# syzhang092218-source/dgppo

Hardware: AMD Instinct MI355X
Metric: env-steps/sec whole node, LidarSpread n=8 4096 envs, 1/2/4/8 GPUs (higher is better)
Workload: dtype f32

## Files before the change

### dgppo_amd/csrc/nn_dense.hip

```cpp
#include "common.h"

using f32x4 = __attribute__((ext_vector_type(4))) float;
#ifdef DGPPO_STAMPS
__device__ unsigned long long g_dstamps[32];
#define DSTAMP(i) do { if (blockIdx.x == 0 && threadIdx.x == 0) g_dstamps[i] = __builtin_amdgcn_s_memtime(); } while (0)
extern "C" int32_t dgppo_debug_stamps_dense(unsigned long long* out) {
  return (int32_t)hipMemcpyFromSymbol(out, HIP_SYMBOL(g_dstamps), sizeof(unsigned long long) * 32);
}
#else
#define DSTAMP(i)
#endif

#define DENSE_ROWS 64

struct DenseArgs {
  const float* X; int ldx;
  const float* W; int ldw;
  const float* bias;
  float* Y; int ldy;
  int M, K, N;
  int act;
  int accumulate;
  int trans_w;
  const float* mask; int ldm;
// ... 335 lines not shown
}

struct DenseBwdWArgs {
  const float* X; int ldx;
  const float* dY; int ldy;
  float* dW; int ldw;
  float* db;
  int M, K, N;
  int rows_per_block;
  float* part;
  int part_stride;
  size_t ws_bytes;
};

#define BW_ROWS 32
template <int NT, int KT>
__global__ void __launch_bounds__(256) dense_bwd_w_kernel(DenseBwdWArgs a) {
  extern __shared__ float sm[];
  constexpr int KTW = (KT + 3) / 4;
  constexpr int Kl = (KT & 1) ? KT * 16 : KT * 16 + 16;
  constexpr int Nl = (NT & 1) ? NT * 16 : NT * 16 + 16;
  constexpr int BUF = BW_ROWS * (Kl + Nl);
  constexpr int XQ = KT * 4, YQ = NT * 4;
  constexpr int PFX = (BW_ROWS * XQ + 255) / 256, PFY = (BW_ROWS * YQ + 255) / 256;
  const int K = a.K, N = a.N;
  const int tid = threadIdx.x, lane = tid & 63, wave = tid >> 6;
  const int li = lane & 15, lq = lane >> 4;
  const int m_begin = blockIdx.x * a.rows_per_block;
  const int m_end = min(a.M, m_begin + a.rows_per_block);
  const bool vec = ((K & 3) == 0) && ((a.ldx & 3) == 0) && ((reinterpret_cast<uintptr_t>(a.X) & 15) == 0) &&
                   ((N & 3) == 0) && ((a.ldy & 3) == 0) && ((reinterpret_cast<uintptr_t>(a.dY) & 15) == 0);
  const int K4 = K >> 2, N4 = N >> 2;
  f32x4 acc[KTW][NT];
#pragma unroll
  for (int i = 0; i < KTW; ++i)
#pragma unroll
    for (int t = 0; t < NT; ++t) acc[i][t] = f32x4{0.f, 0.f, 0.f, 0.f};
  float4 pfx[PFX], pfy[PFY], csum[PFY];
#pragma unroll
  for (int u = 0; u < PFY; ++u) csum[u] = make_float4(0.f, 0.f, 0.f, 0.f);

  auto fetch = [&](int m0) {
#pragma unroll
    for (int u = 0; u < PFX; ++u) {
// ... 62 lines not shown
        av[i] = xs[s4 * 4 * Kl + kt * 16];
      }
#pragma unroll
      for (int i = 0; i < KTW; ++i)
#pragma unroll
        for (int t = 0; t < NT; ++t) acc[i][t] = __builtin_amdgcn_mfma_f32_16x16x4f32(av[i], bv[t], acc[i][t], 0, 0, 0);
    }
  };
#define DGPPO_LDS_BARRIER() asm volatile("s_waitcnt lgkmcnt(0)\n\ts_barrier" ::: "memory")
  float colsum = 0.0f;
  if (vec) {
    fetch(m_begin);
    commit(m_begin, 0);
    __syncthreads();
    int cur = 0;
    for (int m0 = m_begin; m0 < m_end; m0 += BW_ROWS) {
      fetch(m0 + BW_ROWS);
      __builtin_amdgcn_sched_barrier(0);
      compute(cur);
      commit(m0 + BW_ROWS, cur ^ 1);
      DGPPO_LDS_BARRIER();
      cur ^= 1;
    }
  } else {
    for (int m0 = m_begin; m0 < m_end; m0 += BW_ROWS) {
      stage_scalar(m0);
      __syncthreads();
      if (a.db != nullptr && tid < N) {
        const float* ys = sm + BW_ROWS * Kl;
        float cs = 0.0f;
#pragma unroll 8
        for (int r = 0; r < BW_ROWS; ++r) cs += ys[r * Nl + tid];
        colsum += cs;
      }
      compute(0);
      __syncthreads();
    }
  }
#undef DGPPO_LDS_BARRIER
  float* slab = a.part ? a.part + (size_t)blockIdx.x * a.part_stride : nullptr;
#pragma unroll
  for (int i = 0; i < KTW; ++i) {
    const int kt = wave + 4 * i;
    if (kt >= KT) continue;
#pragma unroll
    for (int t = 0; t < NT; ++t) {
      const int col = t * 16 + li;
      if (col >= N) continue;
#pragma unroll
      for (int r = 0; r < 4; ++r) {
        const int krow = kt * 16 + lq * 4 + r;
        if (krow >= K) continue;
        if (slab) slab[krow * N + col] = acc[i][t][r];
        else atomicAdd(a.dW + (size_t)krow * a.ldw + col, acc[i][t][r]);
      }
    }
  }
  if (a.db != nullptr) {
    float cs = colsum;
// ... 1 lines not shown
      __syncthreads();
      float* red = sm;
#pragma unroll
      for (int u = 0; u < PFY; ++u) {
        const int idx = u * 256 + tid;
        const int r = idx / YQ, q = idx - r * YQ;
        if (idx < BW_ROWS * YQ) *reinterpret_cast<float4*>(red + r * (YQ * 4) + 4 * q) = csum[u];
      }
      __syncthreads();
      cs = 0.0f;
      if (tid < N) {
#pragma unroll 8
        for (int r = 0; r < BW_ROWS; ++r) cs += red[r * (YQ * 4) + tid];
      }
    }
    if (tid < N) {
      if (slab) slab[K * N + tid] = cs;
      else atomicAdd(a.db + tid, cs);
    }
  }
}

__global__ void __launch_bounds__(256) dense_bwd_w_reduce_kernel(const float* __restrict__ part, int part_stride, int G,
                                                                 float* __restrict__ dW, int ldw, float* __restrict__ db,
                                                                 int K, int N) {
  const int e = blockIdx.x * 256 + threadIdx.x;
  const int E = K * N + (db ? N : 0);
  if (e >= E) return;
  const int per = (G + gridDim.y - 1) / gridDim.y;
  const int g0 = blockIdx.y * per, g1 = min(G, g0 + per);
  float s0 = 0.f, s1 = 0.f, s2 = 0.f, s3 = 0.f;
  int g = g0;
  for (; g + 3 < g1; g += 4) {
    s0 += part[(size_t)g * part_stride + e];
    s1 += part[(size_t)(g + 1) * part_stride + e];
    s2 += part[(size_t)(g + 2) * part_stride + e];
// ... 11 lines not shown
}

static thread_local dgppo_reduce_desc* g_defer = nullptr;

struct ReduceBatch {
  int n;
  dgppo_reduce_desc d[DGPPO_REDUCE_BATCH];
};

__global__ void __launch_bounds__(256) dense_bwd_w_reduce_batch_kernel(ReduceBatch b) {
  const dgppo_reduce_desc& d = b.d[blockIdx.z];
  const int K = d.K, N = d.N, G = d.slabs;
  const int e = blockIdx.x * 256 + threadIdx.x;
  const int E = K * N + (d.db ? N : 0);
  if (e >= E) return;
  const int splits = min((int)gridDim.y, max(1, (G + 31) / 32));
  if ((int)blockIdx.y >= splits) return;
  const int per = (G + splits - 1) / splits;
  const int g0 = blockIdx.y * per, g1 = min(G, g0 + per);
  if (g0 >= g1) return;
  const float* part = d.part;
  const size_t st = (size_t)d.part_stride;
  float s0 = 0.f, s1 = 0.f, s2 = 0.f, s3 = 0.f;
  int g = g0;
  for (; g + 3 < g1; g += 4) {
    s0 += part[(size_t)g * st + e]; s1 += part[(size_t)(g + 1) * st + e];
    s2 += part[(size_t)(g + 2) * st + e]; s3 += part[(size_t)(g + 3) * st + e];
  }
  for (; g < g1; ++g) s0 += part[(size_t)g * st + e];
  const float sum = (s0 + s1) + (s2 + s3);
  if (e < K * N) {
    const int k = e / N, n = e - k * N;
    atomicAdd(d.dW + (size_t)k * d.ldw + n, sum);
  } else {
    atomicAdd(d.db + (e - K * N), sum);
  }
}

static void reduce_or_defer(hipStream_t s, const float* part, int stride, int grid, float* dW, int ldw, float* db, int K, int N) {
  if (g_defer != nullptr) {
    dgppo_reduce_desc& d = *g_defer;
    d.part = part; d.part_stride = stride; d.slabs = grid; d.dW = dW; d.ldw = ldw; d.db = db; d.K = K; d.N = N; d.pending = 1;
    return;
  }
  const int E = K * N + (db ? N : 0);
  int splits = cdiv(grid, 32);
  splits = splits < 1 ? 1 : (splits > 64 ? 64 : splits);
  hipLaunchKernelGGL(dense_bwd_w_reduce_kernel, dim3(cdiv(E, 256), splits), dim3(256), 0, s, part, stride, grid, dW, ldw, db, K, N);
}

template <int NT, int KT>
static void launch_bwd_w_kt(DenseBwdWArgs a, hipStream_t s) {
  constexpr int Kl = (KT & 1) ? KT * 16 : KT * 16 + 16;
  constexpr int Nl = (NT & 1) ? NT * 16 : NT * 16 + 16;
  constexpr size_t smem = 2 * sizeof(float) * BW_ROWS * (Kl + Nl);
  static_assert(smem <= 160 * 1024, "dense_bwd_w tiles exceed the 160 KB LDS of a gfx950 CU");
  static thread_local int cap = 0;
  if (cap == 0) {
    int per_cu = 0, dev = 0, cus = 256;
    if (smem > 64 * 1024)
      (void)hipFuncSetAttribute(reinterpret_cast<const void*>(&dense_bwd_w_kernel<NT, KT>),
                                hipFuncAttributeMaxDynamicSharedMemorySize, (int)smem);
    if (hipOccupancyMaxActiveBlocksPerMultiprocessor(&per_cu, reinterpret_cast<const void*>(
            &dense_bwd_w_kernel<NT, KT>), 256, smem) != hipSuccess || per_cu < 1) per_cu = 1;
    if (hipGetDevice(&dev) != hipSuccess ||
        hipDeviceGetAttribute(&cus, hipDeviceAttributeMultiprocessorCount, dev) != hipSuccess || cus < 1) cus = 256;
    cap = per_cu * cus;
  }
  int rpb = cdiv(a.M, cap);
  rpb = ((rpb + BW_ROWS - 1) / BW_ROWS) * BW_ROWS;
  if (rpb < 2 * BW_ROWS) rpb = 2 * BW_ROWS;
  const int stride = ((a.K * a.N + a.N + 63) / 64) * 64;
  const size_t ws_bytes = a.ws_bytes;
  float* ws = cdiv(a.M, rpb) > 4 ? a.part : nullptr;
  if (ws) {
    const long max_slabs = (long)(ws_bytes / (sizeof(float) * stride));
    if (max_slabs < 8) ws = nullptr;
    else if (cdiv(a.M, rpb) > max_slabs) rpb = ((cdiv(a.M, (int)max_slabs) + BW_ROWS - 1) / BW_ROWS) * BW_ROWS;
  }
  a.rows_per_block = rpb;
  a.part = ws;
  a.part_stride = stride;
  const int grid = cdiv(a.M, rpb);
  hipLaunchKernelGGL((dense_bwd_w_kernel<NT, KT>), dim3(grid), dim3(256), smem, s, a);
  if (ws) reduce_or_defer(s, ws, stride, grid, a.dW, a.ldw, a.db, a.K, a.N);
}

template <int NT>
static void launch_bwd_w(const DenseBwdWArgs& a, hipStream_t s) {
  const int kt = cdiv(a.K, 16);
  if (kt <= 1) launch_bwd_w_kt<NT, 1>(a, s);
  else if (kt == 2) launch_bwd_w_kt<NT, 2>(a, s);
  else if (kt == 3) launch_bwd_w_kt<NT, 3>(a, s);
  else if (kt == 4) launch_bwd_w_kt<NT, 4>(a, s);
  else if (kt <= 6) launch_bwd_w_kt<NT, 6>(a, s);
  else if (kt <= 8) launch_bwd_w_kt<NT, 8>(a, s);
  else if (kt == 9) launch_bwd_w_kt<NT, 9>(a, s);
  else if (kt <= 12) launch_bwd_w_kt<NT, 12>(a, s);
  else launch_bwd_w_kt<NT, 16>(a, s);
// ... 109 lines not shown
  DGPPO_REQUIRE(a.N <= 192 && a.K <= 256, "dense_bwd_w: N <= 192 and K <= 256 supported (N=%d K=%d)", a.N, a.K);
  DGPPO_REQUIRE(a.X && a.dY && a.dW, "dense_bwd_w: NULL operand");
  DGPPO_REQUIRE(a.ldx >= a.K && a.ldy >= a.N && a.ldw >= a.N, "dense_bwd_w: leading dimensions too small");
  if (a.M == 0) return 0;
  const int nt = cdiv(a.N, 16);
  if (launch_bwd_w_smallk(a, s)) {}
  else if (nt <= 1) launch_bwd_w<1>(a, s);
  else if (nt <= 2) launch_bwd_w<2>(a, s);
  else if (nt <= 4) launch_bwd_w<4>(a, s);
  else if (nt <= 6) launch_bwd_w<6>(a, s);
  else launch_bwd_w<12>(a, s);
  DGPPO_LAUNCH_CHECK();
  return 0;
}

extern "C" int32_t dgppo_dense_fwd(const float* X, int32_t ldx, const float* W, int32_t ldw, const float* bias, float* Y,
                                   int32_t ldy, int32_t M, int32_t K, int32_t N, int32_t act, int32_t accumulate,
                                   int32_t trans_w, const float* relu_mask, int32_t ldm, void* stream) {
  DGPPO_REQUIRE(relu_mask == nullptr || ldm >= N, "dense: mask leading dimension too small");
  DenseArgs a{X, ldx, W, ldw, bias, Y, ldy, M, K, N, act, accumulate, trans_w, relu_mask, ldm};
  return dense_fwd_launch(a, (hipStream_t)stream);
}

extern "C" int32_t dgppo_dense_bwd_w(const float* X, int32_t ldx, const float* dY, int32_t ldy, float* dW, int32_t ldw,
                                     float* db, int32_t M, int32_t K, int32_t N, float* workspace, int64_t workspace_bytes,
                                     void* stream) {
  DGPPO_REQUIRE(workspace_bytes >= 0 && (workspace != nullptr || workspace_bytes == 0), "dense_bwd_w: bad workspace");
  DGPPO_REQUIRE((reinterpret_cast<uintptr_t>(workspace) & 15) == 0, "dense_bwd_w: workspace must be 16-byte aligned");
  DenseBwdWArgs a{X, ldx, dY, ldy, dW, ldw, db, M, K, N, 0, workspace, 0, (size_t)workspace_bytes};
  return dense_bwd_w_launch(a, (hipStream_t)stream);
// ... 17 lines not shown
  DGPPO_REQUIRE(n >= 0 && (n == 0 || descs != nullptr), "dense_bwd_w_reduce_batch: bad arguments");
  for (int32_t i0 = 0; i0 < n; i0 += DGPPO_REDUCE_BATCH) {
    ReduceBatch b;
    b.n = 0;
    int emax = 0, gmax = 0;
    for (int32_t i = i0; i < n && b.n < DGPPO_REDUCE_BATCH; ++i) {
      if (!descs[i].pending) continue;
      DGPPO_REQUIRE(descs[i].part && descs[i].dW && descs[i].slabs >= 1 && descs[i].K >= 1 && descs[i].N >= 1,
                    "dense_bwd_w_reduce_batch: bad descriptor %d", i);
      b.d[b.n++] = descs[i];
      const int E = descs[i].K * descs[i].N + (descs[i].db ? descs[i].N : 0);
      emax = E > emax ? E : emax;
      gmax = descs[i].slabs > gmax ? descs[i].slabs : gmax;
    }
    if (b.n == 0) continue;
    int splits = cdiv(gmax, 32);
    splits = splits < 1 ? 1 : (splits > 64 ? 64 : splits);
    hipLaunchKernelGGL(dense_bwd_w_reduce_batch_kernel, dim3(cdiv(emax, 256), splits, b.n), dim3(256), 0, (hipStream_t)stream, b);
  }
  DGPPO_LAUNCH_CHECK();
  return 0;
}

extern "C" int64_t dgppo_dense_bwd_w_workspace_bytes(int32_t K, int32_t N) {
  if (K < 1 || N < 1) return 0;
  const int64_t stride = (((int64_t)K * N + N + 63) / 64) * 64;
  return stride * 1024 * (int64_t)sizeof(float);
}
```

### dgppo_amd/csrc/nn_elem.hip

```cpp
#include "common.h"

using f32x4 = __attribute__((ext_vector_type(4))) float;

__device__ inline float wave_sum(float v) {
#pragma unroll
  for (int o = 32; o >= 1; o >>= 1) v += __shfl_xor(v, o);
  return v;
}
template <int NV>
__device__ inline void block_atomic_sums(const float (&v)[NV], float* dst) {
  __shared__ float s_red[4][NV];
  const int lane = threadIdx.x & 63, wave = threadIdx.x >> 6;
#pragma unroll
  for (int k = 0; k < NV; ++k) {
    const float w = wave_sum(v[k]);
    if (lane == 0) s_red[wave][k] = w;
  }
  __syncthreads();
  if (threadIdx.x < NV) {
    float t = 0.0f;
    for (int w = 0; w < (int)(blockDim.x >> 6); ++w) t += s_red[w][threadIdx.x];
    atomicAdd(dst + threadIdx.x, t);
  }
}
// ... 108 lines not shown
#define GRU_H 64
#define GRU_WL 194
#define GRU_HL 66

struct GruArgs {
  const float* gi;
  const float* Wh;
  const float* bhn;
  const float* h0;
  float* hs;
  float* hprev;
  float* gates;
  const float* dhs;
  float* dgi;
  float* dgh;
  int n_seq, T, n_inner;
};

__device__ inline size_t gru_row(const GruArgs& a, int s, int tau) {
  const int grp = s / a.n_inner, i = s - grp * a.n_inner;
  return ((size_t)grp * a.T + tau) * a.n_inner + i;
}
__device__ inline float sigmoidf_(float x) { return 1.0f / (1.0f + expf(-x)); }
__device__ inline float gate_sigmoid(float x) { return __builtin_amdgcn_rcpf(1.0f + __expf(-x)); }
__device__ inline float gate_tanh(float x) { return fmaf(2.0f, __builtin_amdgcn_rcpf(1.0f + __expf(-2.0f * x)), -1.0f); }


#define GRU_LDS_BARRIER() asm volatile("s_waitcnt lgkmcnt(0)\n\ts_barrier" ::: "memory")

template <int RTW>
// ... 112 lines not shown
              float* gs = a.gates + row * 256;
              gs[c] = rg; gs[64 + c] = zg; gs[128 + c] = ng; gs[192 + c] = hn;
            }
          }
        }
      GRU_LDS_BARRIER();
      cur ^= 1;
    }
    if (nxt < n_tiles) {
      commit_h0(sm + cur * (RB * GRU_HL));
      GRU_LDS_BARRIER();
    }
  }
}

template <int RTW>
__global__ void __launch_bounds__(256) gru_bwd_kernel(GruArgs a) {
  extern __shared__ float sm[];
  constexpr int RB = 16 * RTW;
  const int tid = threadIdx.x, lane = tid & 63, w = tid >> 6, li = lane & 15, lq = lane >> 4;
  const int c = w * 16 + li;
  float breg[48];
#pragma unroll
  for (int kk = 0; kk < 48; ++kk) breg[kk] = a.Wh[(size_t)c * 192 + kk * 4 + lq];
  const int n_tiles = (a.n_seq + RB - 1) / RB;
  int cur = 0;
  for (int tile = blockIdx.x; tile < n_tiles; tile += gridDim.x) {
    const int s0 = tile * RB;
    int row0[RTW][4];
    bool ok[RTW][4];
#pragma unroll
// ... 36 lines not shown
          const float d = ok[rt][r] ? dh[rt][r] + du[rt][r] : 0.0f;
          const float dz = d * (hp[rt][r] - ng[rt][r]);
          const float dn = d * (1.0f - zg[rt][r]);
          const float dan = dn * (1.0f - ng[rt][r] * ng[rt][r]);
          const float dhn = dan * rg[rt][r];
          const float dar = dan * hn[rt][r] * rg[rt][r] * (1.0f - rg[rt][r]);
          const float daz = dz * zg[rt][r] * (1.0f - zg[rt][r]);
          dh[rt][r] = d * zg[rt][r];
          s_g[rl * GRU_WL + c] = dar;
          s_g[rl * GRU_WL + 64 + c] = daz;
          s_g[rl * GRU_WL + 128 + c] = dhn;
          if (ok[rt][r]) {
            const size_t row = (size_t)(row0[rt][r] + tau * a.n_inner);
            float* o = a.dgi + row * 192 + c;
            o[0] = dar; o[64] = daz; o[128] = dan;
            float* p = a.dgh + row * 192 + c;
            p[0] = dar; p[64] = daz; p[128] = dhn;
          }
        }
      GRU_LDS_BARRIER();
      if (tau > 0) fetch(tau - 1);
      __builtin_amdgcn_sched_barrier(0);
      f32x4 acc[RTW];
#pragma unroll
      for (int rt = 0; rt < RTW; ++rt) acc[rt] = f32x4{0.f, 0.f, 0.f, 0.f};
#pragma unroll
      for (int k0 = 0; k0 < 48; k0 += 16) {
        float areg[RTW][16];
#pragma unroll
        for (int rt = 0; rt < RTW; ++rt)
#pragma unroll
          for (int u = 0; u < 16; ++u) areg[rt][u] = s_g[(rt * 16 + li) * GRU_WL + (k0 + u) * 4 + lq];
// ... 41 lines not shown
    static thread_local int cap = 0;
    if (cap == 0) cap = gru_resident(reinterpret_cast<const void*>(&gru_fwd_kernel<2>), smem);
    const int tiles = cdiv(n_seq, 32);
    hipLaunchKernelGGL(gru_fwd_kernel<2>, dim3(tiles < cap ? tiles : cap), dim3(256), smem, (hipStream_t)stream, a);
  } else {
    const size_t smem = sizeof(float) * 2 * 16 * GRU_HL;
    static thread_local int cap = 0;
    if (cap == 0) cap = gru_resident(reinterpret_cast<const void*>(&gru_fwd_kernel<1>), smem);
    const int tiles = cdiv(n_seq, 16);
    hipLaunchKernelGGL(gru_fwd_kernel<1>, dim3(tiles < cap ? tiles : cap), dim3(256), smem, (hipStream_t)stream, a);
  }
  DGPPO_LAUNCH_CHECK();
  return 0;
}

extern "C" int32_t dgppo_gru_bwd(const float* dhs, const float* Wh, const float* hprev, const float* gates, float* dgi,
                                 float* dgh, int32_t n_seq, int32_t T, int32_t n_inner, void* stream) {
  GruArgs a{};
  a.dhs = dhs; a.Wh = Wh; a.hprev = (float*)hprev; a.gates = (float*)gates; a.dgi = dgi; a.dgh = dgh;
  a.n_seq = n_seq; a.T = T; a.n_inner = n_inner;
  int32_t rc = gru_check(a);
  if (rc) return rc;
  if (n_seq == 0) return 0;
  DGPPO_REQUIRE(dhs && Wh && hprev && gates && dgi && dgh, "gru_bwd: NULL operand");
  if (cdiv(n_seq, 32) >= 512) {
    const size_t smem = sizeof(float) * 2 * 32 * GRU_WL;
    static thread_local int cap = 0;
    if (cap == 0) cap = gru_resident(reinterpret_cast<const void*>(&gru_bwd_kernel<2>), smem);
    const int tiles = cdiv(n_seq, 32);
    hipLaunchKernelGGL(gru_bwd_kernel<2>, dim3(tiles < cap ? tiles : cap), dim3(256), smem, (hipStream_t)stream, a);
  } else {
    const size_t smem = sizeof(float) * 2 * 16 * GRU_WL;
    static thread_local int cap = 0;
    if (cap == 0) cap = gru_resident(reinterpret_cast<const void*>(&gru_bwd_kernel<1>), smem);
    const int tiles = cdiv(n_seq, 16);
    hipLaunchKernelGGL(gru_bwd_kernel<1>, dim3(tiles < cap ? tiles : cap), dim3(256), smem, (hipStream_t)stream, a);
  }
  DGPPO_LAUNCH_CHECK();
  return 0;
}

#define STD_INIT_INV (-0.43275212956718856f)
#define STD_MIN 1e-5f
#define THRESH 0.999f
#define INV_THRESH 3.8002011672502f
#define LOG_EPS (-6.907755278982137f)
#define HALF_LOG_2PI 0.9189385332046727f
#define LOG2_F 0.6931471805599453f

__device__ inline float softplusf_(float x) { return (x > 20.0f) ? x : log1pf(expf(x)); }
#define NDTR_SERIES_BELOW (-10.0f)
__device__ inline float ndtr_tail_series(float z2) { return 1.0f - 1.0f / z2 + 3.0f / (z2 * z2) - 15.0f / (z2 * z2 * z2); }
__device__ inline float log_ndtrf_(float z) {
  if (z > NDTR_SERIES_BELOW) return logf(0.5f * erfcf(-z * 0.70710678118654752f));
// ... 215 lines not shown
```

### dgppo_amd/nets.py

```python
from __future__ import annotations

import math
from typing import Dict, List, Optional, Tuple

import numpy as np
import torch

from . import _native as N
from . import ops_nn as K

H_HEADS = 3
MSG_DIM = 32
OUT_DIM = 64
HID = 64


def _ceil4(x):
    return (x + 3) // 4 * 4


class Layout:
    def __init__(self):
        self.entries: Dict[str, Tuple[int, Tuple[int, ...]]] = {}
        self.size = 0
# ... 240 lines not shown
                saves = tuple(A.get(f"{tag}.{nm}{i}", Rh, w) for i in (1, 2) for nm, w in (("p", HID), ("y", HID), ("st", 2)))
                for i in (1, 2):
                    act[f"p{i}"], act[f"y{i}"], act[f"st{i}"] = saves[3 * (i - 1):3 * i]
            K.mlp_gi_fwd(x, self.p("mlp.W1"), self.p("mlp.b1"), self.p("mlp.g1"), self.p("mlp.be1"), self.p("mlp.W2"),
                         self.p("mlp.b2"), self.p("mlp.g2"), self.p("mlp.be2"), self.p("gru.Wi"), self.p("gru.bi"), gi, saves)
        assert n_seq * T == Rh, (n_seq, T, Rh)
        L, CD = self.rnn_layers, self.carry_dim
        if h0 is not None:
            assert tuple(h0.shape) == (n_seq, CD), (tuple(h0.shape), n_seq, CD)
        if hs_out is not None:
            assert tuple(hs_out.shape) == (Rh, CD), (tuple(hs_out.shape), Rh, CD)
        act["gi"] = gi
        simple = (self.rnn == "gru" and L == 1)
        if simple:
            hs = hs_out if hs_out is not None else A.get(f"{tag}.hs", Rh, HID)
            hprev = A.get(f"{tag}.hprev", Rh, HID) if train else None
            gates = A.get(f"{tag}.gates", Rh, 4 * HID) if train else None
            feat = hs
            act["hs"], act["hprev"], act["gates"] = hs, hprev, gates
        fused_tail = (simple and T == 1 and self.kind == "policy")
        if simple and not fused_tail:
            K.gru_fwd(gi, self.p("gru.Wh"), self.p("gru.bhn"), h0, hs, hprev, gates, n_seq, T, n_inner)
        if self.rnn == "none":
            feat = act["y2"]
            if hs_out is not None:
                if h0 is not None and T == 1:
                    hs_out.copy_(h0)
                else:
                    hs_out.zero_()
        elif self.rnn == "lstm":
            x_l = act["y2"]
            act["stack"] = []
            for l in range(L):
                zi = A.get(f"{tag}.zi{l}", Rh, 4 * HID)
                for half in (slice(0, 2 * HID), slice(2 * HID, 4 * HID)):
                    K.dense_fwd(x_l, self.p(f"lstm{l}.Wi")[:, half], None, zi[:, half])
                c0_l = h0_l = None
# ... 101 lines not shown
        elif self.rnn == "lstm":
            stack = act["stack"]
            for l in range(len(stack) - 1, -1, -1):
                st = stack[l]
                dz = A.get(f"{tag}.dz_lstm{l}", Rh, 4 * HID)
                K.lstm_bwd(dhs, self.p(f"lstm{l}.Wh"), st["cprev"], st["gates"], dz, n_seq, T, n_inner)
                for half in (slice(0, 2 * HID), slice(2 * HID, 4 * HID)):
                    K.dense_bwd_w(st["hprev"], dz[:, half], self.g(f"lstm{l}.Wh")[:, half], self.g(f"lstm{l}.bh")[half])
                    K.dense_bwd_w(st["x"], dz[:, half], self.g(f"lstm{l}.Wi")[:, half], None)
                dx = A.get(f"{tag}.dy" if l == 0 else f"{tag}.dx{l}", Rh, HID)
                K.dense_fwd(dz, self.p(f"lstm{l}.Wi"), None, dx, trans_w=True)
                dhs = dx
            dy = dhs
        else:
            stack = act.get("stack") or [dict(x=None, gi=act["gi"], hs=act["hs"], hprev=act["hprev"], gates=act["gates"])]
            for l in range(len(stack) - 1, -1, -1):
                st = stack[l]
                pre = "gru" if l == 0 else f"gru{l}"
                dgi = A.get(f"{tag}.dgi{l}", Rh, 3 * HID)
                dgh = A.get(f"{tag}.dgh{l}", Rh, 3 * HID)
                K.gru_bwd(dhs, self.p(f"{pre}.Wh"), st["hprev"], st["gates"], dgi, dgh, n_seq, T, n_inner)
                K.dense_bwd_w(st["hprev"], dgh[:, :2 * HID], self.g(f"{pre}.Wh")[:, :2 * HID], None)
                K.dense_bwd_w(st["hprev"], dgh[:, 2 * HID:], self.g(f"{pre}.Wh")[:, 2 * HID:], self.g(f"{pre}.bhn"))
                x_l = act["y2"] if l == 0 else st["x"]
                K.dense_bwd_w(x_l, dgi, self.g(f"{pre}.Wi"), self.g(f"{pre}.bi"))
                if l == 0 and fused_trunk:
                    dgi0 = dgi
                    break
                dx = A.get(f"{tag}.dy" if l == 0 else f"{tag}.dx{l}", Rh, HID)
                K.dense_fwd(dgi, self.p(f"{pre}.Wi"), None, dx, trans_w=True)
# ... 152 lines not shown
```

### dgppo_amd/ops_nn.py

```python
from __future__ import annotations

import ctypes as C
from typing import Optional

import torch

from . import _native as N

FLOPS = [0.0]


def _mat(t: torch.Tensor, name: str):
    if t.dim() != 2:
        raise ValueError(f"{name} must be 2-D, got {tuple(t.shape)}")
    if not t.is_cuda:
        raise RuntimeError(f"{name} must live on the GPU (the HIP path has no CPU fallback)")
    if t.dtype != torch.float32:
        raise TypeError(f"{name} must be float32")
    if t.shape[1] > 1 and t.stride(1) != 1:
        raise ValueError(f"{name} must have unit inner stride")
    ld = t.stride(0) if t.shape[0] > 1 else max(t.shape[1], t.stride(0))
    return C.c_void_p(t.data_ptr()), int(ld), int(t.shape[0]), int(t.shape[1])


# ... 353 lines not shown
    rc = N.lib().dgppo_gru_fwd(_p(gi), _p(Wh), _p(bhn), _p(h0), _p(hs), _p(hprev), _p(gates), n_seq, T, n_inner,
                               N.stream_ptr())
    N.check(rc, "dgppo_gru_fwd")


def gru_bwd(dhs, Wh, hprev, gates, dgi, dgh, n_seq, T, n_inner):
    rows = n_seq * T
    N.expect_shape(dhs, (rows, 64), "dhs")
    N.expect_shape(dgi, (rows, 192), "dgi")
    N.expect_shape(dgh, (rows, 192), "dgh")
    FLOPS[0] += 2.0 * rows * 64 * 192
    rc = N.lib().dgppo_gru_bwd(_p(dhs), _p(Wh), _p(hprev), _p(gates), _p(dgi), _p(dgh), n_seq, T, n_inner, N.stream_ptr())
    N.check(rc, "dgppo_gru_bwd")


def policy_head(ms, eps, action_in, action, log_pi, entropy, n_agents, mode, log_pi_old=None, adv=None, dms=None,
                stats=None, clip_eps=0.25, coef_ent=0.01):
    rows = ms.shape[0]
    N.expect_shape(ms, (rows, 4), "ms")
    rc = N.lib().dgppo_policy_head(_p(ms), _p(eps), _p(action_in), _p(action), _p(log_pi), _p(entropy), rows, n_agents,
                                   mode, _p(log_pi_old), _p(adv), _p(dms), _p(stats), C.c_float(clip_eps),
                                   C.c_float(coef_ent), N.stream_ptr())
    N.check(rc, "dgppo_policy_head")


def value_loss(v, target, dv, stats):
    rc = N.lib().dgppo_value_loss(_p(v), _p(target), _p(dv), _p(stats), v.numel(), N.stream_ptr())
    N.check(rc, "dgppo_value_loss")


# ... 30 lines not shown
```

### include/dgppo_hip.h

```cpp
#ifndef DGPPO_HIP_H
#define DGPPO_HIP_H

#include <stdint.h>

#ifdef __cplusplus
extern "C" {
#endif

#define DGPPO_ABI_VERSION 3

enum {
  DGPPO_ENV_LIDAR_SPREAD = 0,
  DGPPO_ENV_LIDAR_TARGET = 1,
  DGPPO_ENV_LIDAR_BICYCLE_TARGET = 2,
  DGPPO_ENV_MPE_SPREAD = 3,
  DGPPO_ENV_MPE_TARGET = 4,
  DGPPO_ENV_LIDAR_LINE = 5,
  DGPPO_ENV_MPE_LINE = 6,
  DGPPO_ENV_MPE_FORMATION = 7,
  DGPPO_ENV_MPE_CORRIDOR = 8,
  DGPPO_ENV_MPE_CONNECT_SPREAD = 9,
  DGPPO_ENV_VMAS_REVERSE_TRANSPORT = 10
};
enum {
// ... 149 lines not shown
                       const float* We, const float* Wu, float* Mcat, float* cvec, float* Wout, int32_t F, int32_t Fp,
                       int32_t D, int32_t H, int32_t Kp, void* stream);
int32_t dgppo_gnn_unprep(const float* dMcat, const float* dcvec, const float* dWout, const float* Wq, const float* bq,
                         const float* Wk, float* dWq, float* dbq, float* dWk, float* dWv, float* dbv, float* dWe,
                         float* dWu, int32_t F, int32_t Fp, int32_t D, int32_t H, int32_t Kp, void* stream);

int32_t dgppo_ln_relu_fwd(const float* x, const float* gamma, const float* beta, float* y, float* stats, int32_t M,
                          void* stream);
int32_t dgppo_ln_relu_bwd(const float* x, const float* y, const float* stats, const float* gamma, const float* dy,
                          float* dx, float* dgamma, float* dbeta, int32_t M, void* stream);

int32_t dgppo_gru_fwd(const float* gi, const float* Wh, const float* bhn, const float* h0, float* hs, float* hprev,
                      float* gates, int32_t n_seq, int32_t T, int32_t n_inner, void* stream);
int32_t dgppo_gru_bwd(const float* dhs, const float* Wh, const float* hprev, const float* gates, float* dgi,
                      float* dgh, int32_t n_seq, int32_t T, int32_t n_inner, void* stream);

int32_t dgppo_lstm_fwd(const float* zi, const float* Wh, const float* bh, const float* c0, const float* h0, float* cs,
                       float* hs, float* cprev, float* hprev, float* gates, int32_t n_seq, int32_t T, int32_t n_inner,
                       void* stream);
int32_t dgppo_lstm_bwd(const float* dhs, const float* Wh, const float* cprev, const float* gates, float* dz,
                       int32_t n_seq, int32_t T, int32_t n_inner, void* stream);

int32_t dgppo_policy_head(const float* ms, const float* eps, const float* action_in, float* action, float* log_pi,
                          float* entropy, int32_t rows, int32_t n_agents, int32_t mode, const float* log_pi_old,
                          const float* adv, float* dms, float* stats, float clip_eps, float coef_ent, void* stream);

int32_t dgppo_value_loss(const float* v, const float* target, float* dv, float* stats, int32_t count, void* stream);
int32_t dgppo_mean_agents(const float* x, float* y, int32_t G, int32_t n, int32_t D, int32_t backward,
                          const float* relu_mask, void* stream);
int32_t dgppo_relu_bwd(float* dy, const float* y, int64_t count, void* stream);
// ... 36 lines not shown
```

Measured before the change: 4.004 million.

## Add fused GRU weight-gradient kernel, multi-group bwd_w blocks, and reuse h0 as hprev

Adds a dedicated GRU backward weight-gradient kernel that computes dWi, dWh and both bias gradients in one pass from x, hprev, dgi and dhn. It also adds a dhn-only GRU backward variant feeding it, so the separate dense weight-gradient launches for the GRU go away. The generic dense_bwd_w kernel can now pack several 256-thread groups per workgroup and combine their partials through LDS before writing slabs, which cuts the number of partial slabs to reduce. The reduce split size is halved, and when T==1 the stored hprev buffer is replaced by aliasing h0. This adds code paths and LDS pressure, and moves floating-point summation order.

```diff
diff --git a/dgppo_amd/csrc/nn_dense.hip b/dgppo_amd/csrc/nn_dense.hip
--- a/dgppo_amd/csrc/nn_dense.hip
+++ b/dgppo_amd/csrc/nn_dense.hip
@@ -373,9 +373,9 @@
 };
 
 #define BW_ROWS 32
-template <int NT, int KT>
-__global__ void __launch_bounds__(256) dense_bwd_w_kernel(DenseBwdWArgs a) {
-  extern __shared__ float sm[];
+template <int NT, int KT, int NG>
+__global__ void __launch_bounds__(256 * NG) dense_bwd_w_kernel(DenseBwdWArgs a) {
+  extern __shared__ float sm_wg[];
   constexpr int KTW = (KT + 3) / 4;
   constexpr int Kl = (KT & 1) ? KT * 16 : KT * 16 + 16;
   constexpr int Nl = (NT & 1) ? NT * 16 : NT * 16 + 16;
@@ -383,10 +383,14 @@
   constexpr int XQ = KT * 4, YQ = NT * 4;
   constexpr int PFX = (BW_ROWS * XQ + 255) / 256, PFY = (BW_ROWS * YQ + 255) / 256;
   const int K = a.K, N = a.N;
-  const int tid = threadIdx.x, lane = tid & 63, wave = tid >> 6;
+  const int grp = NG > 1 ? (int)(threadIdx.x >> 8) : 0;
+  const int tid = threadIdx.x & 255, lane = tid & 63, wave = tid >> 6;
   const int li = lane & 15, lq = lane >> 4;
-  const int m_begin = blockIdx.x * a.rows_per_block;
+  float* sm = sm_wg + grp * 2 * BUF;
+  const int wg_begin = blockIdx.x * NG * a.rows_per_block;
+  const int m_begin = wg_begin + grp * a.rows_per_block;
   const int m_end = min(a.M, m_begin + a.rows_per_block);
+  const int n_tiles = (min(a.M - wg_begin, a.rows_per_block) + BW_ROWS - 1) / BW_ROWS;
   const bool vec = ((K & 3) == 0) && ((a.ldx & 3) == 0) && ((reinterpret_cast<uintptr_t>(a.X) & 15) == 0) &&
                    ((N & 3) == 0) && ((a.ldy & 3) == 0) && ((reinterpret_cast<uintptr_t>(a.dY) & 15) == 0);
   const int K4 = K >> 2, N4 = N >> 2;
@@ -479,7 +483,7 @@
     commit(m_begin, 0);
     __syncthreads();
     int cur = 0;
-    for (int m0 = m_begin; m0 < m_end; m0 += BW_ROWS) {
+    for (int it = 0, m0 = m_begin; it < n_tiles; ++it, m0 += BW_ROWS) {
       fetch(m0 + BW_ROWS);
       __builtin_amdgcn_sched_barrier(0);
       compute(cur);
@@ -488,7 +492,7 @@
       cur ^= 1;
     }
   } else {
-    for (int m0 = m_begin; m0 < m_end; m0 += BW_ROWS) {
+    for (int it = 0, m0 = m_begin; it < n_tiles; ++it, m0 += BW_ROWS) {
       stage_scalar(m0);
       __syncthreads();
       if (a.db != nullptr && tid < N) {
@@ -503,11 +507,50 @@
     }
   }
 #undef DGPPO_LDS_BARRIER
+  if (NG > 1) {
+    constexpr int ACCF = KTW * NT * 4 * 256;
+    static_assert(NG == 1 || ACCF + PFY * 4 * 256 <= 2 * BUF, "dense_bwd_w: the group exchange does not fit the tile buffers");
+    __syncthreads();
+    if (grp > 0) {
+#pragma unroll
+      for (int i = 0; i < KTW; ++i)
+#pragma unroll
+        for (int t = 0; t < NT; ++t)
+#pragma unroll
+          for (int r = 0; r < 4; ++r) sm[((i * NT + t) * 4 + r) * 256 + tid] = acc[i][t][r];
+      if (!vec) csum[0].x = colsum;
+#pragma unroll
+      for (int u = 0; u < PFY; ++u) {
+        sm[ACCF + (u * 4 + 0) * 256 + tid] = csum[u].x; sm[ACCF + (u * 4 + 1) * 256 + tid] = csum[u].y;
+        sm[ACCF + (u * 4 + 2) * 256 + tid] = csum[u].z; sm[ACCF + (u * 4 + 3) * 256 + tid] = csum[u].w;
+      }
+    }
+    __syncthreads();
+    if (grp == 0) {
+      for (int g = 1; g < NG; ++g) {
+        const float* o = sm_wg + g * 2 * BUF;
+#pragma unroll
+        for (int i = 0; i < KTW; ++i)
+#pragma unroll
+          for (int t = 0; t < NT; ++t)
+#pragma unroll
+            for (int r = 0; r < 4; ++r) acc[i][t][r] += o[((i * NT + t) * 4 + r) * 256 + tid];
+        if (!vec) colsum += o[ACCF + tid];
+        else {
+#pragma unroll
+          for (int u = 0; u < PFY; ++u) {
+            csum[u].x += o[ACCF + (u * 4 + 0) * 256 + tid]; csum[u].y += o[ACCF + (u * 4 + 1) * 256 + tid];
+            csum[u].z += o[ACCF + (u * 4 + 2) * 256 + tid]; csum[u].w += o[ACCF + (u * 4 + 3) * 256 + tid];
+          }
+        }
+      }
+    }
+  }
   float* slab = a.part ? a.part + (size_t)blockIdx.x * a.part_stride : nullptr;
 #pragma unroll
   for (int i = 0; i < KTW; ++i) {
     const int kt = wave + 4 * i;
-    if (kt >= KT) continue;
+    if (kt >= KT || grp != 0) continue;
 #pragma unroll
     for (int t = 0; t < NT; ++t) {
       const int col = t * 16 + li;
@@ -539,12 +582,14 @@
         for (int r = 0; r < BW_ROWS; ++r) cs += red[r * (YQ * 4) + tid];
       }
     }
-    if (tid < N) {
+    if (tid < N && grp == 0) {
       if (slab) slab[K * N + tid] = cs;
       else atomicAdd(a.db + tid, cs);
     }
   }
 }
+
+#define REDUCE_SLABS_PER_SPLIT 16
 
 __global__ void __launch_bounds__(256) dense_bwd_w_reduce_kernel(const float* __restrict__ part, int part_stride, int G,
                                                                  float* __restrict__ dW, int ldw, float* __restrict__ db,
@@ -586,7 +631,7 @@
   const int e = blockIdx.x * 256 + threadIdx.x;
   const int E = K * N + (d.db ? N : 0);
   if (e >= E) return;
-  const int splits = min((int)gridDim.y, max(1, (G + 31) / 32));
+  const int splits = min((int)gridDim.y, max(1, (G + REDUCE_SLABS_PER_SPLIT - 1) / REDUCE_SLABS_PER_SPLIT));
   if ((int)blockIdx.y >= splits) return;
   const int per = (G + splits - 1) / splits;
   const int g0 = blockIdx.y * per, g1 = min(G, g0 + per);
@@ -616,9 +661,31 @@
     return;
   }
   const int E = K * N + (db ? N : 0);
-  int splits = cdiv(grid, 32);
+  int splits = cdiv(grid, REDUCE_SLABS_PER_SPLIT);
   splits = splits < 1 ? 1 : (splits > 64 ? 64 : splits);
   hipLaunchKernelGGL(dense_bwd_w_reduce_kernel, dim3(cdiv(E, 256), splits), dim3(256), 0, s, part, stride, grid, dW, ldw, db, K, N);
+}
+
+static int device_cus() {
+  static thread_local int cus = 0;
+  if (cus == 0) {
+    int dev = 0;
+    if (hipGetDevice(&dev) != hipSuccess ||
+        hipDeviceGetAttribute(&cus, hipDeviceAttributeMultiprocessorCount, dev) != hipSuccess || cus < 1) cus = 256;
+  }
+  return cus;
+}
+
+template <int NT, int KT>
+constexpr int bwd_w_groups() {
+  constexpr int KTW = (KT + 3) / 4;
+  constexpr int Kl = (KT & 1) ? KT * 16 : KT * 16 + 16;
+  constexpr int Nl = (NT & 1) ? NT * 16 : NT * 16 + 16;
+  constexpr int BUF2 = 2 * BW_ROWS * (Kl + Nl);
+  constexpr int PFY = (BW_ROWS * NT * 4 + 255) / 256;
+  constexpr int fit = (160 * 1024) / (BUF2 * 4);
+  constexpr bool xch = KTW * NT * 4 * 256 + PFY * 4 * 256 <= BUF2;
+  return (!xch || fit < 2) ? 1 : (fit > 4 ? 4 : fit);
 }
 
 template <int NT, int KT>
@@ -626,35 +693,37 @@
   constexpr int Kl = (KT & 1) ? KT * 16 : KT * 16 + 16;
   constexpr int Nl = (NT & 1) ? NT * 16 : NT * 16 + 16;
   constexpr size_t smem = 2 * sizeof(float) * BW_ROWS * (Kl + Nl);
-  static_assert(smem <= 160 * 1024, "dense_bwd_w tiles exceed the 160 KB LDS of a gfx950 CU");
-  static thread_local int cap = 0;
-  if (cap == 0) {
-    int per_cu = 0, dev = 0, cus = 256;
+  constexpr int NG = bwd_w_groups<NT, KT>();
+  static_assert(smem * NG <= 160 * 1024, "dense_bwd_w tiles exceed the 160 KB LDS of a gfx950 CU");
+  static thread_local bool opted = false;
+  if (!opted) {
     if (smem > 64 * 1024)
-      (void)hipFuncSetAttribute(reinterpret_cast<const void*>(&dense_bwd_w_kernel<NT, KT>),
+      (void)hipFuncSetAttribute(reinterpret_cast<const void*>(&dense_bwd_w_kernel<NT, KT, 1>),
                                 hipFuncAttributeMaxDynamicSharedMemorySize, (int)smem);
-    if (hipOccupancyMaxActiveBlocksPerMultiprocessor(&per_cu, reinterpret_cast<const void*>(
-            &dense_bwd_w_kernel<NT, KT>), 256, smem) != hipSuccess || per_cu < 1) per_cu = 1;
-    if (hipGetDevice(&dev) != hipSuccess ||
-        hipDeviceGetAttribute(&cus, hipDeviceAttributeMultiprocessorCount, dev) != hipSuccess || cus < 1) cus = 256;
-    cap = per_cu * cus;
-  }
-  int rpb = cdiv(a.M, cap);
+    if (NG > 1 && smem * NG > 64 * 1024)
+      (void)hipFuncSetAttribute(reinterpret_cast<const void*>(&dense_bwd_w_kernel<NT, KT, NG>),
+                                hipFuncAttributeMaxDynamicSharedMemorySize, (int)(smem * NG));
+    opted = true;
+  }
+  const int cus = device_cus();
+  int rpb = cdiv(a.M, NG * cus);
   rpb = ((rpb + BW_ROWS - 1) / BW_ROWS) * BW_ROWS;
   if (rpb < 2 * BW_ROWS) rpb = 2 * BW_ROWS;
+  const int ng = cdiv(a.M, rpb) > cus ? NG : 1;
   const int stride = ((a.K * a.N + a.N + 63) / 64) * 64;
   const size_t ws_bytes = a.ws_bytes;
   float* ws = cdiv(a.M, rpb) > 4 ? a.part : nullptr;
   if (ws) {
     const long max_slabs = (long)(ws_bytes / (sizeof(float) * stride));
     if (max_slabs < 8) ws = nullptr;
-    else if (cdiv(a.M, rpb) > max_slabs) rpb = ((cdiv(a.M, (int)max_slabs) + BW_ROWS - 1) / BW_ROWS) * BW_ROWS;
+    else if (cdiv(a.M, rpb * ng) > max_slabs) rpb = ((cdiv(a.M, (int)max_slabs * ng) + BW_ROWS - 1) / BW_ROWS) * BW_ROWS;
   }
   a.rows_per_block = rpb;
   a.part = ws;
   a.part_stride = stride;
-  const int grid = cdiv(a.M, rpb);
-  hipLaunchKernelGGL((dense_bwd_w_kernel<NT, KT>), dim3(grid), dim3(256), smem, s, a);
+  const int grid = cdiv(a.M, rpb * ng);
+  if (NG > 1 && ng > 1) hipLaunchKernelGGL((dense_bwd_w_kernel<NT, KT, NG>), dim3(grid), dim3(256 * NG), smem * NG, s, a);
+  else hipLaunchKernelGGL((dense_bwd_w_kernel<NT, KT, 1>), dim3(grid), dim3(256), smem, s, a);
   if (ws) reduce_or_defer(s, ws, stride, grid, a.dW, a.ldw, a.db, a.K, a.N);
 }
 
@@ -794,6 +863,182 @@
   return 0;
 }
 
+#define GW_AL 144
+#define GW_YL 272
+#define GW_BUF (BW_ROWS * (GW_AL + GW_YL))
+#define GW_SLAB_WI 0
+#define GW_SLAB_BI (64 * 192)
+#define GW_SLAB_WH (64 * 192 + 192)
+#define GW_SLAB_BHN (2 * 64 * 192 + 192)
+#define GW_SLAB (2 * 64 * 192 + 192 + 64)
+struct GruBwdWArgs {
+  const float* x; int ldx;
+  const float* hprev; int ldh;
+  const float* dgi;
+  const float* dhn;
+  float* dWi; int ldwi;
+  float* dbi;
+  float* dWh; int ldwh;
+  float* dbhn;
+  int M, rows_per_block;
+  float* part;
+};
+
+__global__ void __launch_bounds__(512) gru_bwd_w_kernel(GruBwdWArgs a) {
+  extern __shared__ float sm[];
+  const int tid = threadIdx.x, lane = tid & 63, wave = (tid >> 6) & 3, half = tid >> 8;
+  const int li = lane & 15, lq = lane >> 4;
+  const int m_begin = blockIdx.x * a.rows_per_block;
+  const int m_end = min(a.M, m_begin + a.rows_per_block);
+  f32x4 acc[12];
+#pragma unroll
+  for (int t = 0; t < 12; ++t) acc[t] = f32x4{0.f, 0.f, 0.f, 0.f};
+  float4 pfa[2], pfy[4];
+  float4 csum = make_float4(0.f, 0.f, 0.f, 0.f);
+  const int qa = tid & 31, ra = tid >> 5, qy = tid & 63, ry = tid >> 6;
+  auto fetch = [&](int m0) {
+#pragma unroll
+    for (int u = 0; u < 2; ++u) {
+      int row = m0 + u * 16 + ra;
+      row = row < a.M ? row : a.M - 1;
+      const float* src = qa < 16 ? a.x + (size_t)row * a.ldx + 4 * qa : a.hprev + (size_t)row * a.ldh + 4 * (qa - 16);
+      pfa[u] = *reinterpret_cast<const float4*>(src);
+    }
+#pragma unroll
+    for (int u = 0; u < 4; ++u) {
+      int row = m0 + u * 8 + ry;
+      row = row < a.M ? row : a.M - 1;
+      const float* src = qy < 48 ? a.dgi + (size_t)row * 192 + 4 * qy : a.dhn + (size_t)row * 64 + 4 * (qy - 48);
+      pfy[u] = *reinterpret_cast<const float4*>(src);
+    }
+  };
+  auto commit = [&](int m0, int b) {
+    float* as = sm + b * GW_BUF;
+    float* ys = as + BW_ROWS * GW_AL;
+#pragma unroll
+    for (int u = 0; u < 2; ++u) {
+      const int r = u * 16 + ra;
+      const float4 v = (m0 + r < m_end) ? pfa[u] : make_float4(0.f, 0.f, 0.f, 0.f);
+      *reinterpret_cast<float4*>(as + r * GW_AL + 4 * qa) = v;
+    }
+#pragma unroll
+    for (int u = 0; u < 4; ++u) {
+      const int r = u * 8 + ry;
+      const float4 v = (m0 + r < m_end) ? pfy[u] : make_float4(0.f, 0.f, 0.f, 0.f);
+      *reinterpret_cast<float4*>(ys + r * GW_YL + 4 * qy) = v;
+      csum.x += v.x; csum.y += v.y; csum.z += v.z; csum.w += v.w;
+    }
+  };
+  auto compute = [&](int b) {
+    const float* as = sm + b * GW_BUF + lq * GW_AL + half * 64 + wave * 16 + li;
+    const float* ys = sm + b * GW_BUF + BW_ROWS * GW_AL + lq * GW_YL + li;
+    const float* yh = ys + (half ? 64 : 0);
+#pragma unroll
+    for (int s4 = 0; s4 < BW_ROWS / 4; ++s4) {
+      float bv[12];
+#pragma unroll
+      for (int t = 0; t < 8; ++t) bv[t] = ys[s4 * 4 * GW_YL + t * 16];
+#pragma unroll
+      for (int t = 8; t < 12; ++t) bv[t] = yh[s4 * 4 * GW_YL + t * 16];
+      const float av = as[s4 * 4 * GW_AL];
+#pragma unroll
+      for (int t = 0; t < 12; ++t) acc[t] = __builtin_amdgcn_mfma_f32_16x16x4f32(av, bv[t], acc[t], 0, 0, 0);
+    }
+  };
+  fetch(m_begin);
+  commit(m_begin, 0);
+  __syncthreads();
+  int cur = 0;
+  for (int m0 = m_begin; m0 < m_end; m0 += BW_ROWS) {
+    fetch(m0 + BW_ROWS);
+    __builtin_amdgcn_sched_barrier(0);
+    compute(cur);
+    commit(m0 + BW_ROWS, cur ^ 1);
+    asm volatile("s_waitcnt lgkmcnt(0)\n\ts_barrier" ::: "memory");
+    cur ^= 1;
+  }
+  float* slab = a.part ? a.part + (size_t)blockIdx.x * GW_SLAB : nullptr;
+  {
+    float* out = half ? a.dWh : a.dWi;
+    const int ldo = half ? a.ldwh : a.ldwi;
+    float* sl = slab ? slab + (half ? GW_SLAB_WH : GW_SLAB_WI) : nullptr;
+#pragma unroll
+    for (int t = 0; t < 12; ++t) {
+      const int col = t * 16 + li;
+#pragma unroll
+      for (int r = 0; r < 4; ++r) {
+        const int krow = wave * 16 + lq * 4 + r;
+        if (sl) sl[krow * 192 + col] = acc[t][r];
+        else atomicAdd(out + (size_t)krow * ldo + col, acc[t][r]);
+      }
+    }
+  }
+  __syncthreads();
+  *reinterpret_cast<float4*>(sm + ry * 256 + 4 * qy) = csum;
+  __syncthreads();
+  if (tid < 256) {
+    float cs = 0.0f;
+#pragma unroll
+    for (int r = 0; r < 8; ++r) cs += sm[r * 256 + tid];
+    if (tid < 192) {
+      if (slab) slab[GW_SLAB_BI + tid] = cs;
+      else atomicAdd(a.dbi + tid, cs);
+    } else {
+      if (slab) slab[GW_SLAB_BHN + tid - 192] = cs;
+      else atomicAdd(a.dbhn + tid - 192, cs);
+    }
+  }
+}
+
+extern "C" int64_t dgppo_gru_bwd_w_workspace_bytes(void) { return (int64_t)GW_SLAB * sizeof(float) * device_cus(); }
+
+extern "C" int32_t dgppo_gru_bwd_w(const float* x, int32_t ldx, const float* hprev, int32_t ldh, const float* dgi,
+                                   const float* dhn, float* dWi, int32_t ldwi, float* dbi, float* dWh, int32_t ldwh,
+                                   float* dbhn, int32_t M, float* workspace, int64_t workspace_bytes,
+                                   dgppo_reduce_desc* pending, void* stream) {
+  DGPPO_REQUIRE(M >= 0, "gru_bwd_w: bad M");
+  DGPPO_REQUIRE(x && hprev && dgi && dhn && dWi && dbi && dWh && dbhn, "gru_bwd_w: NULL operand");
+  DGPPO_REQUIRE(ldx >= 64 && ldh >= 64 && ldwi >= 192 && ldwh >= 192, "gru_bwd_w: leading dimensions too small");
+  DGPPO_REQUIRE((ldx & 3) == 0 && (ldh & 3) == 0 && ((reinterpret_cast<uintptr_t>(x) | reinterpret_cast<uintptr_t>(hprev) |
+                 reinterpret_cast<uintptr_t>(dgi) | reinterpret_cast<uintptr_t>(dhn)) & 15) == 0,
+                "gru_bwd_w: x, hprev, dgi, dhn must be 16-byte aligned with leading dimensions that are multiples of 4");
+  DGPPO_REQUIRE(workspace_bytes >= 0 && (workspace != nullptr || workspace_bytes == 0), "gru_bwd_w: bad workspace");
+  DGPPO_REQUIRE((reinterpret_cast<uintptr_t>(workspace) & 15) == 0, "gru_bwd_w: workspace must be 16-byte aligned");
+  if (pending) pending[0].pending = pending[1].pending = pending[2].pending = 0;
+  if (M == 0) return 0;
+  hipStream_t s = (hipStream_t)stream;
+  constexpr size_t smem = 2 * sizeof(float) * GW_BUF;
+  static_assert(smem <= 160 * 1024, "gru_bwd_w tiles exceed the 160 KB LDS of a gfx950 CU");
+  static thread_local bool opted = false;
+  if (!opted) {
+    (void)hipFuncSetAttribute(reinterpret_cast<const void*>(&gru_bwd_w_kernel), hipFuncAttributeMaxDynamicSharedMemorySize, (int)smem);
+    opted = true;
+  }
+  int rpb = cdiv(M, device_cus());
+  rpb = ((rpb + BW_ROWS - 1) / BW_ROWS) * BW_ROWS;
+  if (rpb < 2 * BW_ROWS) rpb = 2 * BW_ROWS;
+  float* ws = cdiv(M, rpb) > 4 ? workspace : nullptr;
+  if (ws) {
+    const long max_slabs = (long)(workspace_bytes / (sizeof(float) * GW_SLAB));
+    if (max_slabs < 8) ws = nullptr;
+    else if (cdiv(M, rpb) > max_slabs) rpb = ((cdiv(M, (int)max_slabs) + BW_ROWS - 1) / BW_ROWS) * BW_ROWS;
+  }
+  const int grid = cdiv(M, rpb);
+  GruBwdWArgs a{x, ldx, hprev, ldh, dgi, dhn, dWi, ldwi, dbi, dWh, ldwh, dbhn, M, rpb, ws};
+  hipLaunchKernelGGL(gru_bwd_w_kernel, dim3(grid), dim3(512), smem, s, a);
+  DGPPO_LAUNCH_CHECK();
+  if (!ws) return 0;
+  dgppo_reduce_desc d[3];
+  d[0] = dgppo_reduce_desc{ws + GW_SLAB_WI, dWi, dbi, GW_SLAB, grid, ldwi, 64, 192, 1};
+  d[1] = dgppo_reduce_desc{ws + GW_SLAB_WH, dWh, nullptr, GW_SLAB, grid, ldwh, 64, 192, 1};
+  d[2] = dgppo_reduce_desc{ws + GW_SLAB_BHN, dbhn, nullptr, GW_SLAB, grid, 64, 1, 64, 1};
+  if (pending) {
+    pending[0] = d[0]; pending[1] = d[1]; pending[2] = d[2];
+    return 0;
+  }
+  return dgppo_dense_bwd_w_reduce_batch(d, 3, stream);
+}
+
 extern "C" int32_t dgppo_dense_fwd(const float* X, int32_t ldx, const float* W, int32_t ldw, const float* bias, float* Y,
                                    int32_t ldy, int32_t M, int32_t K, int32_t N, int32_t act, int32_t accumulate,
                                    int32_t trans_w, const float* relu_mask, int32_t ldm, void* stream) {
@@ -841,7 +1086,7 @@
       gmax = descs[i].slabs > gmax ? descs[i].slabs : gmax;
     }
     if (b.n == 0) continue;
-    int splits = cdiv(gmax, 32);
+    int splits = cdiv(gmax, REDUCE_SLABS_PER_SPLIT);
     splits = splits < 1 ? 1 : (splits > 64 ? 64 : splits);
     hipLaunchKernelGGL(dense_bwd_w_reduce_batch_kernel, dim3(cdiv(emax, 256), splits, b.n), dim3(256), 0, (hipStream_t)stream, b);
   }
diff --git a/dgppo_amd/csrc/nn_elem.hip b/dgppo_amd/csrc/nn_elem.hip
--- a/dgppo_amd/csrc/nn_elem.hip
+++ b/dgppo_amd/csrc/nn_elem.hip
@@ -146,6 +146,7 @@
   const float* dhs;
   float* dgi;
   float* dgh;
+  float* dhn;
   int n_seq, T, n_inner;
 };
 
@@ -288,7 +289,7 @@
   }
 }
 
-template <int RTW>
+template <int RTW, bool DHN_ONLY>
 __global__ void __launch_bounds__(256) gru_bwd_kernel(GruArgs a) {
   extern __shared__ float sm[];
   constexpr int RB = 16 * RTW;
@@ -355,8 +356,12 @@
             const size_t row = (size_t)(row0[rt][r] + tau * a.n_inner);
             float* o = a.dgi + row * 192 + c;
             o[0] = dar; o[64] = daz; o[128] = dan;
-            float* p = a.dgh + row * 192 + c;
-            p[0] = dar; p[64] = daz; p[128] = dhn;
+            if (DHN_ONLY) {
+              a.dhn[row * GRU_H + c] = dhn;
+            } else {
+              float* p = a.dgh + row * 192 + c;
+              p[0] = dar; p[64] = daz; p[128] = dhn;
+            }
           }
         }
       GRU_LDS_BARRIER();
@@ -428,30 +433,43 @@
   return 0;
 }
 
+template <bool DHN_ONLY>
+static int32_t gru_bwd_launch(GruArgs a, hipStream_t stream) {
+  int32_t rc = gru_check(a);
+  if (rc) return rc;
+  if (a.n_seq == 0) return 0;
+  DGPPO_REQUIRE(a.dhs && a.Wh && a.hprev && a.gates && a.dgi && (DHN_ONLY ? a.dhn : a.dgh), "gru_bwd: NULL operand");
+  if (cdiv(a.n_seq, 32) >= 512) {
+    const size_t smem = sizeof(float) * 2 * 32 * GRU_WL;
+    static thread_local int cap = 0;
+    if (cap == 0) cap = gru_resident(reinterpret_cast<const void*>(&gru_bwd_kernel<2, DHN_ONLY>), smem);
+    const int tiles = cdiv(a.n_seq, 32);
+    hipLaunchKernelGGL((gru_bwd_kernel<2, DHN_ONLY>), dim3(tiles < cap ? tiles : cap), dim3(256), smem, stream, a);
+  } else {
+    const size_t smem = sizeof(float) * 2 * 16 * GRU_WL;
+    static thread_local int cap = 0;
+    if (cap == 0) cap = gru_resident(reinterpret_cast<const void*>(&gru_bwd_kernel<1, DHN_ONLY>), smem);
+    const int tiles = cdiv(a.n_seq, 16);
+    hipLaunchKernelGGL((gru_bwd_kernel<1, DHN_ONLY>), dim3(tiles < cap ? tiles : cap), dim3(256), smem, stream, a);
+  }
+  DGPPO_LAUNCH_CHECK();
+  return 0;
+}
+
 extern "C" int32_t dgppo_gru_bwd(const float* dhs, const float* Wh, const float* hprev, const float* gates, float* dgi,
                                  float* dgh, int32_t n_seq, int32_t T, int32_t n_inner, void* stream) {
   GruArgs a{};
   a.dhs = dhs; a.Wh = Wh; a.hprev = (float*)hprev; a.gates = (float*)gates; a.dgi = dgi; a.dgh = dgh;
   a.n_seq = n_seq; a.T = T; a.n_inner = n_inner;
-  int32_t rc = gru_check(a);
-  if (rc) return rc;
-  if (n_seq == 0) return 0;
-  DGPPO_REQUIRE(dhs && Wh && hprev && gates && dgi && dgh, "gru_bwd: NULL operand");
-  if (cdiv(n_seq, 32) >= 512) {
-    const size_t smem = sizeof(float) * 2 * 32 * GRU_WL;
-    static thread_local int cap = 0;
-    if (cap == 0) cap = gru_resident(reinterpret_cast<const void*>(&gru_bwd_kernel<2>), smem);
-    const int tiles = cdiv(n_seq, 32);
-    hipLaunchKernelGGL(gru_bwd_kernel<2>, dim3(tiles < cap ? tiles : cap), dim3(256), smem, (hipStream_t)stream, a);
-  } else {
-    const size_t smem = sizeof(float) * 2 * 16 * GRU_WL;
-    static thread_local int cap = 0;
-    if (cap == 0) cap = gru_resident(reinterpret_cast<const void*>(&gru_bwd_kernel<1>), smem);
-    const int tiles = cdiv(n_seq, 16);
-    hipLaunchKernelGGL(gru_bwd_kernel<1>, dim3(tiles < cap ? tiles : cap), dim3(256), smem, (hipStream_t)stream, a);
-  }
-  DGPPO_LAUNCH_CHECK();
-  return 0;
+  return gru_bwd_launch<false>(a, (hipStream_t)stream);
+}
+
+extern "C" int32_t dgppo_gru_bwd_dhn(const float* dhs, const float* Wh, const float* hprev, const float* gates, float* dgi,
+                                     float* dhn, int32_t n_seq, int32_t T, int32_t n_inner, void* stream) {
+  GruArgs a{};
+  a.dhs = dhs; a.Wh = Wh; a.hprev = (float*)hprev; a.gates = (float*)gates; a.dgi = dgi; a.dhn = dhn;
+  a.n_seq = n_seq; a.T = T; a.n_inner = n_inner;
+  return gru_bwd_launch<true>(a, (hipStream_t)stream);
 }
 
 #define STD_INIT_INV (-0.43275212956718856f)
diff --git a/dgppo_amd/nets.py b/dgppo_amd/nets.py
--- a/dgppo_amd/nets.py
+++ b/dgppo_amd/nets.py
@@ -278,13 +278,16 @@
         simple = (self.rnn == "gru" and L == 1)
         if simple:
             hs = hs_out if hs_out is not None else A.get(f"{tag}.hs", Rh, HID)
-            hprev = A.get(f"{tag}.hprev", Rh, HID) if train else None
+            hprev_is_h0 = train and T == 1 and h0 is not None and self.kind != "policy"
+            hprev = A.get(f"{tag}.hprev", Rh, HID) if (train and not hprev_is_h0) else None
             gates = A.get(f"{tag}.gates", Rh, 4 * HID) if train else None
             feat = hs
             act["hs"], act["hprev"], act["gates"] = hs, hprev, gates
         fused_tail = (simple and T == 1 and self.kind == "policy")
         if simple and not fused_tail:
             K.gru_fwd(gi, self.p("gru.Wh"), self.p("gru.bhn"), h0, hs, hprev, gates, n_seq, T, n_inner)
+            if hprev_is_h0:
+                act["hprev"] = h0
         if self.rnn == "none":
             feat = act["y2"]
             if hs_out is not None:
@@ -416,6 +419,18 @@
             dy = dhs
         else:
             stack = act.get("stack") or [dict(x=None, gi=act["gi"], hs=act["hs"], hprev=act["hprev"], gates=act["gates"])]
+            if act.get("stack") is None and dout.is_cuda:
+                st = stack[0]
+                dgi = A.get(f"{tag}.dgi0", Rh, 3 * HID)
+                dhn = A.get(f"{tag}.dhn0", Rh, HID)
+                K.gru_bwd_dhn(dhs, self.p("gru.Wh"), st["hprev"], st["gates"], dgi, dhn, n_seq, T, n_inner)
+                K.gru_bwd_w(act["y2"], st["hprev"], dgi, dhn, self.g("gru.Wi"), self.g("gru.bi"), self.g("gru.Wh"), self.g("gru.bhn"))
+                if fused_trunk:
+                    dgi0 = dgi
+                else:
+                    dhs = A.get(f"{tag}.dy", Rh, HID)
+                    K.dense_fwd(dgi, self.p("gru.Wi"), None, dhs, trans_w=True)
+                stack = []
             for l in range(len(stack) - 1, -1, -1):
                 st = stack[l]
                 pre = "gru" if l == 0 else f"gru{l}"
diff --git a/dgppo_amd/ops_nn.py b/dgppo_amd/ops_nn.py
--- a/dgppo_amd/ops_nn.py
+++ b/dgppo_amd/ops_nn.py
@@ -391,6 +391,50 @@
     N.check(rc, "dgppo_gru_bwd")
 
 
+def gru_bwd_dhn(dhs, Wh, hprev, gates, dgi, dhn, n_seq, T, n_inner):
+    rows = n_seq * T
+    N.expect_shape(dhs, (rows, 64), "dhs")
+    N.expect_shape(dgi, (rows, 192), "dgi")
+    N.expect_shape(dhn, (rows, 64), "dhn")
+    FLOPS[0] += 2.0 * rows * 64 * 192
+    rc = N.lib().dgppo_gru_bwd_dhn(_p(dhs), _p(Wh), _p(hprev), _p(gates), _p(dgi), _p(dhn), n_seq, T, n_inner, N.stream_ptr())
+    N.check(rc, "dgppo_gru_bwd_dhn")
+
+
+def gru_bwd_w(x, hprev, dgi, dhn, dWi, dbi, dWh, dbhn):
+    xp, ldx, M, Kx = _mat(x, "x")
+    hp, ldh, Mh, Kh = _mat(hprev, "hprev")
+    wip, ldwi, _, _ = _mat(dWi, "dWi")
+    whp, ldwh, _, _ = _mat(dWh, "dWh")
+    if Kx != 64 or (Mh, Kh) != (M, 64) or tuple(dWi.shape) != (64, 192) or tuple(dWh.shape) != (64, 192):
+        raise ValueError(f"gru_bwd_w: shape mismatch x{tuple(x.shape)} hprev{tuple(hprev.shape)} dWi{tuple(dWi.shape)} "
+                         f"dWh{tuple(dWh.shape)}")
+    N.expect_shape(dgi, (M, 192), "dgi"); N.expect_shape(dhn, (M, 64), "dhn")
+    N.expect_shape(dbi, (192,), "dbi"); N.expect_shape(dbhn, (64,), "dbhn")
+    FLOPS[0] += 2.0 * M * 64 * (128 + 64 + 192)
+    lib = N.lib()
+    lib.dgppo_gru_bwd_w_workspace_bytes.restype = C.c_int64
+    need = int(lib.dgppo_gru_bwd_w_workspace_bytes())
+    batch = BwdWBatch._active.get((x.device.index, torch.cuda.current_stream(x.device).cuda_stream)) if x.is_cuda else None
+    if batch is not None:
+        ws = batch.region(need)
+        d = (ReduceDesc * 3)()
+        pend = d
+    else:
+        key = (x.device.index, torch.cuda.current_stream(x.device).cuda_stream, "gru")
+        ws = _WS.get(key)
+        if ws is None or ws.numel() * 4 < need:
+            ws = _WS[key] = torch.empty(need // 4, dtype=torch.float32, device=x.device)
+        pend = None
+    rc = lib.dgppo_gru_bwd_w(xp, ldx, hp, ldh, _p(dgi, "dgi"), _p(dhn, "dhn"), wip, ldwi, _p(dbi, "dbi"), whp, ldwh,
+                             _p(dbhn, "dbhn"), M, _p(ws, "workspace"), C.c_int64(ws.numel() * 4), pend, N.stream_ptr())
+    N.check(rc, "dgppo_gru_bwd_w")
+    if batch is not None:
+        for i in range(3):
+            if d[i].pending:
+                batch.descs.append(ReduceDesc.from_buffer_copy(d[i]))
+
+
 def policy_head(ms, eps, action_in, action, log_pi, entropy, n_agents, mode, log_pi_old=None, adv=None, dms=None,
                 stats=None, clip_eps=0.25, coef_ent=0.01):
     rows = ms.shape[0]
diff --git a/include/dgppo_hip.h b/include/dgppo_hip.h
--- a/include/dgppo_hip.h
+++ b/include/dgppo_hip.h
@@ -187,6 +187,12 @@
                       float* gates, int32_t n_seq, int32_t T, int32_t n_inner, void* stream);
 int32_t dgppo_gru_bwd(const float* dhs, const float* Wh, const float* hprev, const float* gates, float* dgi,
                       float* dgh, int32_t n_seq, int32_t T, int32_t n_inner, void* stream);
+int32_t dgppo_gru_bwd_dhn(const float* dhs, const float* Wh, const float* hprev, const float* gates, float* dgi,
+                          float* dhn, int32_t n_seq, int32_t T, int32_t n_inner, void* stream);
+int64_t dgppo_gru_bwd_w_workspace_bytes(void);
+int32_t dgppo_gru_bwd_w(const float* x, int32_t ldx, const float* hprev, int32_t ldh, const float* dgi, const float* dhn,
+                        float* dWi, int32_t ldwi, float* dbi, float* dWh, int32_t ldwh, float* dbhn, int32_t M,
+                        float* workspace, int64_t workspace_bytes, dgppo_reduce_desc* pending, void* stream);
 
 int32_t dgppo_lstm_fwd(const float* zi, const float* Wh, const float* bh, const float* c0, const float* h0, float* cs,
                        float* hs, float* cprev, float* hprev, float* gates, int32_t n_seq, int32_t T, int32_t n_inner,
```

New measurement: 4.094 million, median of 6. 1.02x the previous value.
